# alibaba/EasyParallelLibrary

Measured on AMD Instinct MI355X. Metric: samples_per_sec, higher is better.
Workload: dtype bf16; 1 GPU; model=bert-large, global_batch=128, seq_len=512, parallelism=dp1

## Files before the change

### csrc/bindings.hip

```cpp

#include <hip/hip_runtime.h>
#include <torch/extension.h>
#include <ATen/hip/impl/HIPStreamMasqueradingAsCUDA.h>

#include <cstdint>

namespace epl {
void register_comm(py::module& m);
}

extern "C" {
void epl_fused_adamw(float*, unsigned short*, const void*, bool, float*,
                     float*, int64_t, float, float, float, float, float, int,
                     float, hipStream_t);
void epl_lamb_phase1(const float*, const void*, bool, float*, float*, float*,
                     const int*, float*, float*, int64_t, float, float, float,
                     float, int, float, hipStream_t);
void epl_lamb_phase2(float*, unsigned short*, const float*, const int*,
                     const float*, int64_t, float, hipStream_t);
void epl_layer_norm_fwd(void*, const void*, const void*, void*, const void*,
                        const void*, float*, float*, int64_t, int64_t, float,
                        bool, hipStream_t);
void epl_layer_norm_bwd(void*, float*, float*, const void*, const void*,
                        const void*, const float*, const float*, float*,
// ... 11 lines not shown
                       hipStream_t);
void epl_ce_rowstats(const void*, const int64_t*, float*, float*, float*,
                     int64_t, int64_t, int64_t, int64_t, bool, hipStream_t);
void epl_ce_backward(void*, const void*, const int64_t*, const float*,
                     const float*, const float*, int64_t, int64_t, int64_t,
                     int64_t, float, bool, hipStream_t);
void epl_scale(void*, int64_t, float, bool, hipStream_t);
void epl_f32_to_bf16(unsigned short*, const float*, int64_t, hipStream_t);
void epl_bf16_to_f32(float*, const unsigned short*, int64_t, hipStream_t);
void epl_sqnorm(const void*, int64_t, float*, bool, hipStream_t);
void epl_colsum(void*, const void*, float*, int64_t, int64_t, int64_t,
                bool, hipStream_t);
void run_mfma_probe(const unsigned short*, const unsigned short*, float*,
                    hipStream_t);
void run_tr_read_probe(short*, short*, int, hipStream_t);
void epl_moe_dispatch_fwd(void*, const void*, const int64_t*,
                          const int64_t*, const int64_t*, int64_t, int64_t,
                          int64_t, hipStream_t);
void epl_moe_dispatch_bwd(void*, const void*, const int64_t*,
                          const int64_t*, const int64_t*, int64_t, int64_t,
                          int64_t, int64_t, hipStream_t);
void epl_moe_combine_fwd(void*, const void*, const float*, const int64_t*,
                         const int64_t*, const int64_t*, int64_t, int64_t,
                         int64_t, int64_t, hipStream_t);
void epl_moe_combine_bwd(void*, float*, const void*, const void*,
                         const float*, const int64_t*, const int64_t*,
                         const int64_t*, int64_t, int64_t, int64_t,
                         hipStream_t);
int64_t epl_moe_router_waves(int64_t, int64_t);
void epl_moe_router_fwd(const void*, int64_t*, float*, float*, int64_t*,
// ... 405 lines not shown
}

void tr_read_probe(at::Tensor out_gather, at::Tensor out_tr,
                   int64_t head_dim) {
  TORCH_CHECK(head_dim == 64 || head_dim == 128, "head_dim must be 64|128");
  check(out_gather, at::kShort, "out_gather");
  check(out_tr, at::kShort, "out_tr");
  const int64_t n = 4 * (head_dim / 32) * 64 * 8;
  TORCH_CHECK(out_gather.numel() == n && out_tr.numel() == n,
              "probe outputs must hold ", n, " elements");
  run_tr_read_probe(reinterpret_cast<short*>(out_gather.data_ptr()),
                    reinterpret_cast<short*>(out_tr.data_ptr()),
                    (int)head_dim, cur_stream());
}

void mfma_probe(at::Tensor A, at::Tensor B, at::Tensor D) {
  check(A, at::kBFloat16, "A");
  check(B, at::kBFloat16, "B");
  check(D, at::kFloat, "D");
  run_mfma_probe(reinterpret_cast<const unsigned short*>(A.data_ptr()),
                 reinterpret_cast<const unsigned short*>(B.data_ptr()),
                 D.data_ptr<float>(), cur_stream());
}

static void check_idx(const at::Tensor& t, const char* name) {
  TORCH_CHECK(t.is_cuda() && t.is_contiguous() &&
              t.scalar_type() == at::kLong, name,
              " must be a contiguous int64 device tensor");
}

// ... 308 lines not shown
  m.def("layer_norm_bwd", &layer_norm_bwd);
  m.def("layer_norm_bwd_fused", &layer_norm_bwd_fused, py::arg("dx"),
        py::arg("dgamma"), py::arg("dbeta"), py::arg("dy"), py::arg("x"),
        py::arg("gamma"), py::arg("mean"), py::arg("rstd"),
        py::arg("dadd") = py::none(), py::arg("colsum_out") = py::none());
  m.def("bias_gelu_fwd", &bias_gelu_fwd);
  m.def("bias_gelu_bwd", &bias_gelu_bwd);
  m.def("ce_rowstats", &ce_rowstats);
  m.def("ce_backward", &ce_backward);
  m.def("scale_", &scale_);
  m.def("f32_to_bf16", &f32_to_bf16);
  m.def("bf16_to_f32", &bf16_to_f32);
  m.def("sqnorm", &sqnorm);
  m.def("mfma_probe", &mfma_probe);
  m.def("tr_read_probe", &tr_read_probe);
  m.def("moe_dispatch_fwd", &moe_dispatch_fwd);
  m.def("moe_dispatch_bwd", &moe_dispatch_bwd);
  m.def("moe_combine_fwd", &moe_combine_fwd);
  m.def("moe_combine_bwd", &moe_combine_bwd);
  m.def("moe_router_fwd", &moe_router_fwd);
  m.def("moe_router_bwd", &moe_router_bwd);
  m.def("moe_router_waves", [](int64_t n, int64_t e) {
    return epl_moe_router_waves(n, e);
  });
  m.def("attn_fwd", &attn_fwd, py::arg("q"), py::arg("k"), py::arg("v"),
        py::arg("out"), py::arg("lse"), py::arg("scale"), py::arg("causal"),
        py::arg("drop_mask"), py::arg("seed"), py::arg("drop_thresh"),
        py::arg("inv_keep"), py::arg("seqlens") = py::none());
  m.def("attn_bwd", &attn_bwd, py::arg("q"), py::arg("k"), py::arg("v"),
        py::arg("out"), py::arg("dout"), py::arg("lse"),
// ... 16 lines not shown
```

### csrc/kernels/attention.hip

```cpp

#include <hip/hip_runtime.h>
#include <cstdint>
#include <cstdlib>
#include <cstring>
#include <type_traits>

#include "attn_lds_image.h"

using bf16x8 = __attribute__((ext_vector_type(8))) short;
using bf16x4 = __attribute__((ext_vector_type(4))) short;
using f32x16 = __attribute__((ext_vector_type(16))) float;
using i32x2 = __attribute__((ext_vector_type(2))) int;
using u32x2 = __attribute__((ext_vector_type(2))) unsigned int;
using f32x2 = __attribute__((ext_vector_type(2))) float;
using f32x4 = __attribute__((ext_vector_type(4))) float;
using bf16v2 = __attribute__((ext_vector_type(2))) __bf16;

#define DEVI __device__ __forceinline__

namespace {

DEVI float bf2f(short u) {
  union { unsigned int i; float f; } v;
  v.i = ((unsigned int)(unsigned short)u) << 16;
// ... 72 lines not shown
};

DEVI void store_acc_bf16(short* p, const f32x16& acc, int hi) {
#pragma unroll
  for (int g = 0; g < 4; ++g) {
    u32x2 v = {cvt_pk_bf16(acc[4 * g], acc[4 * g + 1]),
               cvt_pk_bf16(acc[4 * g + 2], acc[4 * g + 3])};
    *reinterpret_cast<u32x2*>(p + 8 * g + 4 * hi) = v;
  }
}

DEVI int64_t sample_len(const int* seqlens, int64_t b, int64_t seq) {
  if (seqlens == nullptr) return seq;
  const int64_t n = __builtin_amdgcn_readfirstlane(seqlens[b]);
  return n < 0 ? 0 : (n > seq ? seq : n);
}

template <int D>
DEVI void zero_row(short* p, int hi) {
  const u32x2 z = {0u, 0u};
#pragma unroll
  for (int j = 0; j < D / 32; ++j)
#pragma unroll
    for (int g = 0; g < 4; ++g)
      *reinterpret_cast<u32x2*>(p + j * 32 + 8 * g + 4 * hi) = z;
}

DEVI void philox_round(unsigned int& c0, unsigned int& c1,
                       unsigned int& c2, unsigned int& c3,
                       unsigned int k0, unsigned int k1) {
// ... 119 lines not shown
    const short* __restrict__ q, const short* __restrict__ k,
    const short* __restrict__ v, short* __restrict__ out,
    float* __restrict__ lse, int64_t seq, float scale, int causal,
    int64_t heads, int64_t in_sb, int64_t in_sh, int64_t in_ss,
    int64_t o_sb, int64_t o_sh, int64_t o_ss,
    unsigned int* __restrict__ mask, int64_t mask_w,
    unsigned long long seed, int drop_thresh, float inv_keep,
    const int* __restrict__ seqlens) {
  __shared__ __attribute__((aligned(16))) short
      ldsV[2][64 * img_pitch<D>()];
  __shared__ __attribute__((aligned(16))) short ldsK[2][64][D + 8];
  const int lane = threadIdx.x & 63;
  const int wave = threadIdx.x >> 6;
  const int hi = lane >> 5;
  const int lq = lane & 31;
  const int64_t bh = causal ? (int64_t)blockIdx.x : (int64_t)blockIdx.y;
  const int64_t boff = (bh / heads) * in_sb + (bh % heads) * in_sh;
  const int64_t qb = causal ? (int64_t)gridDim.y - 1 - blockIdx.y
                            : (int64_t)blockIdx.x;
  const int64_t q0_blk = qb * 128;
  const int64_t q0 = q0_blk + wave * 32;
  const int64_t len = sample_len(seqlens, bh / heads, seq);
  const int64_t myq = q0 + lq;
  if (myq >= len && myq < seq) {
    zero_row<D>(out + (bh / heads) * o_sb + (bh % heads) * o_sh +
                    myq * o_ss, hi);
    if (hi == 0) lse[bh * seq + myq] = 0.f;
  }
  if (q0_blk >= len) return;
  const bool active = q0 < len;
  const short* qp = q + boff;
  const short* kp = k + boff;
  const short* vp = v + boff;

  const int64_t qrow = myq < len ? myq : len - 1;
// ... 97 lines not shown
#pragma unroll
  for (int j = 0; j < D / 32; ++j)
    store_acc_bf16(ldsO + lq * (D + 8) + j * 32, ot[j] * inv_l, hi);
  __syncthreads();
  constexpr int LPR = D / 8;
#pragma unroll
  for (int r0 = 0; r0 < 32; r0 += 64 / LPR) {
    const int r = r0 + lane / LPR;
    const int col = (lane % LPR) * 8;
    const bf16x8 piece =
        *reinterpret_cast<const bf16x8*>(ldsO + r * (D + 8) + col);
    if (q0 + r < len)
      *reinterpret_cast<bf16x8*>(ob + (q0 + r) * o_ss + col) = piece;
  }
  if (hi == 0 && myq < len) lse[bh * seq + myq] = m * scale + __logf(l);
}

__global__ void attn_bwd_prep_kernel(const short* __restrict__ dout,
                                     const short* __restrict__ out,
                                     float* __restrict__ delta,
                                     int64_t rows, int64_t seq,
                                     int64_t heads, int64_t do_sb,
                                     int64_t do_sh, int64_t do_ss,
                                     int64_t o_sb, int64_t o_sh,
                                     int64_t o_ss) {
  const int lane = threadIdx.x & 63;
  const int waves_per_block = blockDim.x >> 6;
  for (int64_t row = (int64_t)blockIdx.x * waves_per_block +
                     (threadIdx.x >> 6);
       row < rows; row += (int64_t)gridDim.x * waves_per_block) {
    const int64_t bh = row / seq;
    const int64_t sq = row % seq;
    const short* dp = dout + (bh / heads) * do_sb + (bh % heads) * do_sh +
                      sq * do_ss;
    const short* op = out + (bh / heads) * o_sb + (bh % heads) * o_sh +
                      sq * o_ss;
    float acc = bf2f(dp[lane]) * bf2f(op[lane]);
#pragma unroll
    for (int off = 32; off > 0; off >>= 1)
      acc += __shfl_down(acc, off, 64);
    if (lane == 0) delta[row] = acc;
  }
}

__global__ __launch_bounds__(256) void attn_bwd_dkdv_kernel(
    const short* __restrict__ q, const short* __restrict__ k,
    const short* __restrict__ v, const short* __restrict__ dout,
    const float* __restrict__ lse, const float* __restrict__ delta,
    short* __restrict__ dk, short* __restrict__ dv, int64_t seq,
    float scale, int causal, int64_t heads, int64_t in_sb, int64_t in_sh,
    int64_t in_ss, int64_t do_sb, int64_t do_sh, int64_t do_ss,
    int64_t g_sb, int64_t g_sh, int64_t g_ss) {
  __shared__ short ldsQ[32][72];
  __shared__ short ldsDO[32][72];
  const int lane = threadIdx.x & 63;
  const int wave = threadIdx.x >> 6;
  const int hi = lane >> 5;
  const int lkv = lane & 31;
  const int64_t bh = blockIdx.y;
  const int64_t kv0_blk = (int64_t)blockIdx.x * 128;
  const int64_t kv0 = kv0_blk + wave * 32;
  const bool active = kv0 < seq;
  const int64_t boff = (bh / heads) * in_sb + (bh % heads) * in_sh;
  const short* qp = q + boff;
  const short* kp = k + boff;
  const short* vp = v + boff;
  const short* dop = dout + (bh / heads) * do_sb + (bh % heads) * do_sh;
  const float* lsep = lse + bh * seq;
  const float* dltp = delta + bh * seq;

  const int64_t mykv = kv0 + lkv;
  const int64_t kvrow = mykv < seq ? mykv : seq - 1;

  bf16x8 kfrag[4], vfrag[4];
#pragma unroll
  for (int c = 0; c < 4; ++c) {
    kfrag[c] = *reinterpret_cast<const bf16x8*>(
        kp + kvrow * in_ss + hi * 8 + 16 * c);
    vfrag[c] = *reinterpret_cast<const bf16x8*>(
        vp + kvrow * in_ss + hi * 8 + 16 * c);
  }

  f32x16 dvt0 = {}, dvt1 = {};
  f32x16 dkt0 = {}, dkt1 = {};

  const int stage_row = threadIdx.x >> 3;
  const int stage_seg = (threadIdx.x & 7) * 8;
  const int64_t q_start = causal ? (kv0_blk / 32) * 32 : 0;
  for (int64_t q0 = q_start; q0 < seq; q0 += 32) {
    __syncthreads();
    {
      int64_t qr = q0 + stage_row;
      if (qr >= seq) qr = seq - 1;
      *reinterpret_cast<bf16x8*>(&ldsQ[stage_row][stage_seg]) =
          *reinterpret_cast<const bf16x8*>(qp + qr * in_ss + stage_seg);
      *reinterpret_cast<bf16x8*>(&ldsDO[stage_row][stage_seg]) =
          *reinterpret_cast<const bf16x8*>(dop + qr * do_ss + stage_seg);
    }
    __syncthreads();
    if (!active || (causal && q0 + 31 < kv0)) continue;
    f32x16 st = {};
    f32x16 dpt = {};
#pragma unroll
    for (int c = 0; c < 4; ++c) {
      bf16x8 qf = *reinterpret_cast<const bf16x8*>(
          &ldsQ[lkv][hi * 8 + 16 * c]);
      bf16x8 dof = *reinterpret_cast<const bf16x8*>(
          &ldsDO[lkv][hi * 8 + 16 * c]);
      st = __builtin_amdgcn_mfma_f32_32x32x16_bf16(qf, kfrag[c], st, 0, 0,
                                                   0);
      dpt = __builtin_amdgcn_mfma_f32_32x32x16_bf16(dof, vfrag[c], dpt, 0,
                                                    0, 0);
    }
    float p[16], ds[16];
#pragma unroll
    for (int r = 0; r < 16; ++r) {
      const int64_t qg = q0 + crow(r, hi);
      const int64_t qgc = qg < seq ? qg : seq - 1;
      float sv = st[r] * scale;
      bool masked = qg >= seq || (causal && mykv > qg) || mykv >= seq;
      float pv = masked ? 0.f : __expf(sv - lsep[qgc]);
      p[r] = pv;
      ds[r] = masked ? 0.f : pv * (dpt[r] - dltp[qgc]) * scale;
    }
    bf16x8 pb0 = assemble_pfrag(&p[0]);
    bf16x8 pb1 = assemble_pfrag(&p[8]);
    bf16x8 db0 = assemble_pfrag(&ds[0]);
    bf16x8 db1 = assemble_pfrag(&ds[8]);
#pragma unroll
    for (int qc = 0; qc < 2; ++qc) {
      bf16x8 dot0, dot1, qt0, qt1;
#pragma unroll
      for (int j = 0; j < 8; ++j) {
        const int qr = qc * 16 + hi * 8 + j;
        dot0[j] = ldsDO[qr][lkv];
        dot1[j] = ldsDO[qr][32 + lkv];
        qt0[j] = ldsQ[qr][lkv];
        qt1[j] = ldsQ[qr][32 + lkv];
      }
      bf16x8 pb = qc == 0 ? pb0 : pb1;
      bf16x8 db = qc == 0 ? db0 : db1;
      dvt0 = __builtin_amdgcn_mfma_f32_32x32x16_bf16(dot0, pb, dvt0, 0, 0,
                                                     0);
      dvt1 = __builtin_amdgcn_mfma_f32_32x32x16_bf16(dot1, pb, dvt1, 0, 0,
                                                     0);
      dkt0 = __builtin_amdgcn_mfma_f32_32x32x16_bf16(qt0, db, dkt0, 0, 0,
                                                     0);
      dkt1 = __builtin_amdgcn_mfma_f32_32x32x16_bf16(qt1, db, dkt1, 0, 0,
                                                     0);
    }
  }

  if (!active || mykv >= seq) return;
  const int64_t goff = (bh / heads) * g_sb + (bh % heads) * g_sh +
                       mykv * g_ss;
  short* dkp = dk + goff;
  short* dvp = dv + goff;
#pragma unroll
  for (int r = 0; r < 16; ++r) {
    dvp[crow(r, hi)] = (short)f2bf(dvt0[r]);
    dvp[32 + crow(r, hi)] = (short)f2bf(dvt1[r]);
    dkp[crow(r, hi)] = (short)f2bf(dkt0[r]);
    dkp[32 + crow(r, hi)] = (short)f2bf(dkt1[r]);
  }
}


template <bool MASKED, bool DROP, int D>
DEVI void dv_tile(const short (&ldsQ)[64][D + 8],
                  const short (&ldsDO)[64][D + 8],
                  int sub, int64_t q0, int64_t seq, int64_t mykv,
                  float scale, int causal, const float* lsep,
                  const bf16x8 (&kfrag)[D / 16], f32x16 (&dvt)[D / 32],
                  int lkv, int hi, const unsigned int* maskrow,
                  int64_t mask_w, float inv_keep) {
  f32x16 st = {};
#pragma unroll
  for (int c = 0; c < D / 16; ++c) {
    bf16x8 qf = *reinterpret_cast<const bf16x8*>(
// ... 209 lines not shown
    int64_t heads, int64_t in_sb, int64_t in_sh, int64_t in_ss,
    int64_t do_sb, int64_t do_sh, int64_t do_ss, int64_t g_sb,
    int64_t g_sh, int64_t g_ss,
    const unsigned int* __restrict__ mask, int64_t mask_w,
    float inv_keep, const int* __restrict__ seqlens) {
  constexpr int PITCH = TR ? img_pitch<D>() : D + 8;
  __shared__ __attribute__((aligned(16))) short
      ldsQ[DBUF ? 2 : 1][64][PITCH];
  __shared__ __attribute__((aligned(16))) short
      ldsDO[DBUF ? 2 : 1][64][PITCH];
  __shared__ __attribute__((aligned(16))) float ldsL[DBUF ? 2 : 1][64];
  const int lane = threadIdx.x & 63;
  const int wave = threadIdx.x >> 6;
  const int hi = lane >> 5;
  const int lkv = lane & 31;
  const int64_t bh = causal ? (int64_t)blockIdx.x : (int64_t)blockIdx.y;
  const int64_t kv0_blk =
      (causal ? (int64_t)blockIdx.y : (int64_t)blockIdx.x) * 128;
  const int64_t kv0 = kv0_blk + wave * 32;
  const int64_t len = sample_len(seqlens, bh / heads, seq);
  const int64_t mykv = kv0 + lkv;
  if (mykv >= len && mykv < seq)
    zero_row<D>(dv + (bh / heads) * g_sb + (bh % heads) * g_sh +
                    mykv * g_ss, hi);
  if (kv0_blk >= len) return;
  const bool active = kv0 < len;
  const int64_t boff = (bh / heads) * in_sb + (bh % heads) * in_sh;
  const short* qp = q + boff;
  const short* kp = k + boff;
  const short* dop = dout + (bh / heads) * do_sb + (bh % heads) * do_sh;
  const float* lsep = lse + bh * seq;

  const int64_t kvrow = mykv < len ? mykv : len - 1;
// ... 170 lines not shown
    int64_t heads, int64_t in_sb, int64_t in_sh, int64_t in_ss,
    int64_t do_sb, int64_t do_sh, int64_t do_ss, int64_t g_sb,
    int64_t g_sh, int64_t g_ss,
    const unsigned int* __restrict__ mask, int64_t mask_w,
    float inv_keep, const int* __restrict__ seqlens) {
  constexpr int PITCH = TR ? img_pitch<D>() : D + 8;
  __shared__ __attribute__((aligned(16))) short
      ldsQ[DBUF ? 2 : 1][64][PITCH];
  __shared__ __attribute__((aligned(16))) short
      ldsDO[DBUF ? 2 : 1][64][PITCH];
  __shared__ __attribute__((aligned(16))) float ldsL[DBUF ? 2 : 1][2][64];
  const int lane = threadIdx.x & 63;
  const int wave = threadIdx.x >> 6;
  const int hi = lane >> 5;
  const int lkv = lane & 31;
  const int64_t bh = causal ? (int64_t)blockIdx.x : (int64_t)blockIdx.y;
  const int64_t kv0_blk =
      (causal ? (int64_t)blockIdx.y : (int64_t)blockIdx.x) * 128;
  const int64_t kv0 = kv0_blk + wave * 32;
  const int64_t len = sample_len(seqlens, bh / heads, seq);
  const int64_t mykv = kv0 + lkv;
  if (mykv >= len && mykv < seq)
    zero_row<D>(dk + (bh / heads) * g_sb + (bh % heads) * g_sh +
                    mykv * g_ss, hi);
  if (kv0_blk >= len) return;
  const bool active = kv0 < len;
  const int64_t boff = (bh / heads) * in_sb + (bh % heads) * in_sh;
  const short* qp = q + boff;
  const short* kp = k + boff;
  const short* vp = v + boff;
  const short* dop = dout + (bh / heads) * do_sb + (bh % heads) * do_sh;
  const float* lsep = lse + bh * seq;
  const float* dltp = delta + bh * seq;
// ... 156 lines not shown
  if (!active || mykv >= len) return;
  short* dkp = dk + (bh / heads) * g_sb + (bh % heads) * g_sh +
               mykv * g_ss;
#pragma unroll
  for (int dj = 0; dj < D / 32; ++dj) {
    if constexpr (TR) {
      store_acc_bf16(dkp + dj * 32, dkt[dj], hi);
    } else {
#pragma unroll
      for (int r = 0; r < 16; ++r)
        dkp[dj * 32 + crow(r, hi)] = (short)f2bf(dkt[dj][r]);
    }
  }
}


template <bool MASKED, bool DROP, int D>
DEVI void dq_tile(const short (&ldsK)[64][D + 8],
                  const short (&ldsVr)[64][D + 8],
                  int sub, int64_t kv0, int64_t seq, int64_t myq,
                  float scale, int causal, float mylse, float mydelta,
                  const bf16x8 (&qfrag)[D / 16],
                  const bf16x8 (&dofrag)[D / 16],
                  f32x16 (&dqt)[D / 32], int lq, int hi,
                  const unsigned int* maskrow, int64_t mask_w,
                  float inv_keep) {
  f32x16 st = {};
  f32x16 dpt = {};
#pragma unroll
  for (int c = 0; c < D / 16; ++c) {
// ... 104 lines not shown
    float scale, int causal, int64_t heads, int64_t in_sb, int64_t in_sh,
    int64_t in_ss, int64_t do_sb, int64_t do_sh, int64_t do_ss,
    int64_t g_sb, int64_t g_sh, int64_t g_ss, int64_t o_sb, int64_t o_sh,
    int64_t o_ss, const unsigned int* __restrict__ mask, int64_t mask_w,
    float inv_keep, const float* __restrict__ dlse,
    const int* __restrict__ seqlens) {
  constexpr int PITCH = TR ? img_pitch<D>() : D + 8;
  __shared__ __attribute__((aligned(16))) short
      ldsK[DBUF ? 2 : 1][64][PITCH];
  __shared__ __attribute__((aligned(16))) short
      ldsVr[DBUF ? 2 : 1][64][PITCH];
  const int lane = threadIdx.x & 63;
  const int wave = threadIdx.x >> 6;
  const int hi = lane >> 5;
  const int lq = lane & 31;
  const int64_t bh = causal ? (int64_t)blockIdx.x : (int64_t)blockIdx.y;
  const int64_t qb = causal ? (int64_t)gridDim.y - 1 - blockIdx.y
                            : (int64_t)blockIdx.x;
  const int64_t q0_blk = qb * 128;
  const int64_t q0 = q0_blk + wave * 32;
  const int64_t len = sample_len(seqlens, bh / heads, seq);
  const int64_t myq = q0 + lq;
  if (myq >= len && myq < seq)
    zero_row<D>(dq + (bh / heads) * g_sb + (bh % heads) * g_sh +
                    myq * g_ss, hi);
  if (q0_blk >= len) return;
  const bool active = q0 < len;
  const int64_t boff = (bh / heads) * in_sb + (bh % heads) * in_sh;
  const short* qp = q + boff;
  const short* kp = k + boff;
  const short* vp = v + boff;
  const short* dop = dout + (bh / heads) * do_sb + (bh % heads) * do_sh;

  const int64_t qrow = myq < len ? myq : len - 1;
// ... 194 lines not shown
                       dim3(256), 0, stream, FWD_ARGS);
  }
#undef FWD_ARGS
}

void epl_attn_bwd(const void* q, const void* k, const void* v,
                  const void* out, const void* dout, const float* lse,
                  float* delta_ws, void* dq, void* dk, void* dv,
                  int64_t batch_heads, int64_t seq, float scale,
                  bool causal, int64_t heads, const int64_t* in_strides,
                  const int64_t* o_strides, const int64_t* do_strides,
                  const int64_t* g_strides, int split_dkdv,
                  const unsigned int* drop_mask, int64_t mask_w,
                  float inv_keep, int64_t head_dim, const float* dlse,
                  const int* seqlens, hipStream_t stream) {
  const int64_t rows = batch_heads * seq;
  const unsigned nqb = (unsigned)((seq + 127) / 128);
  dim3 grid = causal ? dim3((unsigned)batch_heads, nqb)
                     : dim3(nqb, (unsigned)batch_heads);
  if (split_dkdv || drop_mask != nullptr || head_dim == 128 || causal ||
      dlse != nullptr || seqlens != nullptr) {
#define DV_ARGS                                                          \
  reinterpret_cast<const short*>(q), reinterpret_cast<const short*>(k),  \
      reinterpret_cast<const short*>(dout), lse,                         \
      reinterpret_cast<short*>(dv), seq, scale, causal ? 1 : 0, heads,   \
      in_strides[0], in_strides[1], in_strides[2], do_strides[0],        \
      do_strides[1], do_strides[2], g_strides[0], g_strides[1],          \
      g_strides[2], drop_mask, mask_w, inv_keep, seqlens
#define DQ_ARGS                                                          \
  reinterpret_cast<const short*>(q), reinterpret_cast<const short*>(k),  \
      reinterpret_cast<const short*>(v),                                 \
      reinterpret_cast<const short*>(dout), lse, delta_ws,               \
      reinterpret_cast<short*>(dq), reinterpret_cast<const short*>(out), \
      seq, scale, causal ? 1 : 0, heads, in_strides[0], in_strides[1],   \
      in_strides[2], do_strides[0], do_strides[1], do_strides[2],        \
      g_strides[0], g_strides[1], g_strides[2], o_strides[0],            \
      o_strides[1], o_strides[2], drop_mask, mask_w, inv_keep, dlse,     \
// ... 10 lines not shown
      const char* e = getenv("EPL_ATTN_BWD_DBUF");
      return e == nullptr ? -1 : atoi(e);
    }();
    const int mode = dbuf_mode < 0 ? (causal ? 0 : 2) : dbuf_mode;
    const bool dbuf = mode >= 1;
    const bool dbuf_k = mode >= 2;
    const bool dbuf_q = mode >= 3;
    static const bool legacy_tiles = [] {
      const char* e = getenv("EPL_ATTN_BWD_TILES");
      return e != nullptr && strcmp(e, "legacy") == 0;
    }();
    auto launch3 = [&](auto drop_c, auto d_c, auto tr_c) {
      constexpr bool DROP = decltype(drop_c)::value;
      constexpr int D = decltype(d_c)::value;
      constexpr bool TR = decltype(tr_c)::value;
      if (D == 64 && dbuf)
        hipLaunchKernelGGL(
            HIP_KERNEL_NAME(attn_bwd_dv_kernel<DROP, D == 64, D, TR>), grid,
            dim3(256), 0, stream, DV_ARGS);
      else
        hipLaunchKernelGGL(
            HIP_KERNEL_NAME(attn_bwd_dv_kernel<DROP, false, D, TR>), grid,
            dim3(256), 0, stream, DV_ARGS);
      if (D == 64 && dbuf_q)
        hipLaunchKernelGGL(
            HIP_KERNEL_NAME(attn_bwd_dq_kernel<DROP, D == 64, D, TR>), grid,
            dim3(256), 0, stream, DQ_ARGS);
      else
        hipLaunchKernelGGL(
            HIP_KERNEL_NAME(attn_bwd_dq_kernel<DROP, false, D, TR>), grid,
            dim3(256), 0, stream, DQ_ARGS);
      if (D == 64 && dbuf_k)
        hipLaunchKernelGGL(
            HIP_KERNEL_NAME(attn_bwd_dk_kernel<DROP, D == 64, D, TR>), grid,
            dim3(256), 0, stream, DK_ARGS);
      else
        hipLaunchKernelGGL(
            HIP_KERNEL_NAME(attn_bwd_dk_kernel<DROP, false, D, TR>), grid,
            dim3(256), 0, stream, DK_ARGS);
    };
    auto launch2 = [&](auto drop_c, auto d_c) {
      if (legacy_tiles)
        launch3(drop_c, d_c, std::false_type{});
      else
        launch3(drop_c, d_c, std::true_type{});
    };
    using d64 = std::integral_constant<int, 64>;
    using d128 = std::integral_constant<int, 128>;
    if (head_dim == 128) {
      if (drop_mask != nullptr)
        launch2(std::true_type{}, d128{});
      else
        launch2(std::false_type{}, d128{});
    } else if (drop_mask != nullptr) {
      launch2(std::true_type{}, d64{});
    } else {
      launch2(std::false_type{}, d64{});
    }
#undef DV_ARGS
#undef DQ_ARGS
#undef DK_ARGS
    return;
  }
  {
    const int64_t blocks = (rows + 3) / 4;
    hipLaunchKernelGGL(attn_bwd_prep_kernel,
                       dim3((unsigned)(blocks < 4096 ? blocks : 4096)),
                       dim3(256), 0, stream,
                       reinterpret_cast<const short*>(dout),
                       reinterpret_cast<const short*>(out), delta_ws, rows,
                       seq, heads, do_strides[0], do_strides[1],
                       do_strides[2], o_strides[0], o_strides[1],
                       o_strides[2]);
  }
  hipLaunchKernelGGL(attn_bwd_dkdv_kernel, grid, dim3(256), 0, stream,
                     reinterpret_cast<const short*>(q),
                     reinterpret_cast<const short*>(k),
                     reinterpret_cast<const short*>(v),
                     reinterpret_cast<const short*>(dout), lse, delta_ws,
                     reinterpret_cast<short*>(dk),
                     reinterpret_cast<short*>(dv), seq, scale,
                     causal ? 1 : 0, heads, in_strides[0], in_strides[1],
                     in_strides[2], do_strides[0], do_strides[1],
                     do_strides[2], g_strides[0], g_strides[1],
                     g_strides[2]);
  hipLaunchKernelGGL(
      HIP_KERNEL_NAME(attn_bwd_dq_kernel<false, false, 64, true>),
                     grid, dim3(256), 0, stream,
                     reinterpret_cast<const short*>(q),
                     reinterpret_cast<const short*>(k),
                     reinterpret_cast<const short*>(v),
                     reinterpret_cast<const short*>(dout), lse, delta_ws,
                     reinterpret_cast<short*>(dq),
                     reinterpret_cast<const short*>(out), seq, scale,
                     causal ? 1 : 0, heads, in_strides[0], in_strides[1],
                     in_strides[2], do_strides[0], do_strides[1],
                     do_strides[2], g_strides[0], g_strides[1],
                     g_strides[2], o_strides[0], o_strides[1],
                     o_strides[2], drop_mask, mask_w, inv_keep, dlse,
                     (const int*)nullptr);
}

}
```

### csrc/kernels/mfma_probe.hip

```cpp

#include <hip/hip_runtime.h>

#include "attn_lds_image.h"

using bf16x8 = __attribute__((ext_vector_type(8))) short;
using f32x16 = __attribute__((ext_vector_type(16))) float;

__global__ void mfma_probe_kernel(const unsigned short* __restrict__ A,
                                  const unsigned short* __restrict__ B,
                                  float* __restrict__ D) {
  const int lane = threadIdx.x & 63;
  const int half = lane >> 5;
  const int lm = lane & 31;
  bf16x8 a, b;
  for (int j = 0; j < 8; ++j) {
    a[j] = (short)A[lm * 16 + (half * 8 + j)];
    b[j] = (short)B[(half * 8 + j) * 32 + lm];
  }
  f32x16 c = {};
  c = __builtin_amdgcn_mfma_f32_32x32x16_bf16(a, b, c, 0, 0, 0);
  for (int reg = 0; reg < 16; ++reg) {
    const int row = (reg & 3) + 8 * (reg >> 2) + 4 * half;
    const int col = lm;
    D[row * 32 + col] = c[reg];
// ... 28 lines not shown
        const bf16x8 t = attn_img::tr_frag<D>(img, sub + qc * 16, dj, lane);
        *reinterpret_cast<bf16x8*>(out_gather + (frag * 64 + lane) * 8) = g;
        *reinterpret_cast<bf16x8*>(out_tr + (frag * 64 + lane) * 8) = t;
      }
}

extern "C" void run_tr_read_probe(short* out_gather, short* out_tr,
                                  int head_dim, hipStream_t stream) {
  if (head_dim == 128)
    hipLaunchKernelGGL(tr_read_probe_kernel<128>, dim3(1), dim3(64), 0,
                       stream, out_gather, out_tr);
  else
    hipLaunchKernelGGL(tr_read_probe_kernel<64>, dim3(1), dim3(64), 0,
                       stream, out_gather, out_tr);
}
```

### easyparallellibrary_amd/ops/attention.py

```python

import torch
import torch.nn.functional as F

from easyparallellibrary_amd.ops.dispatch import native_ext, use_native
from easyparallellibrary_amd.utils.logging import get_logger

logger = get_logger()
_warned = set()


def _warn_fallback(reason):
    if reason not in _warned:
        _warned.add(reason)
        logger.warning(
            "native attention unavailable (%s): falling back to torch "
            "SDPA for these shapes", reason)


def _kernel_ok(t):
    return (t.dim() == 4 and t.shape[-1] in (64, 128)
            and t.stride(-1) == 1
            and t.stride(1) % 8 == 0 and t.stride(2) % 8 == 0)


# ... 14 lines not shown
    if seqlens is None:
        return None
    if seqlens.dtype != torch.int32 or seqlens.dim() != 1 \
            or seqlens.shape[0] != q.shape[0]:
        raise ValueError("seqlens must be int32 [B={}], got {} {}".format(
            q.shape[0], seqlens.dtype, tuple(seqlens.shape)))
    if seqlens.device != q.device:
        raise ValueError("seqlens must be on the device of q")
    return seqlens.contiguous()


def _mask_tensor(b, h, seq, device):
    mask_w = (seq + 31) // 32
    return torch.empty(b * h * seq * mask_w, dtype=torch.int32,
                       device=device)


def _saved_optionals(ctx, rest):
    rest = list(rest)
    mask = rest.pop(0) if ctx.has_mask else None
    seqlens = rest.pop(0) if ctx.has_seqlens else None
    return mask, seqlens


class _FlashAttention(torch.autograd.Function):

    @staticmethod
    def forward(ctx, q, k, v, causal, scale, dropout_p=0.0, seqlens=None):
        if not (_kernel_ok(q) and _kernel_ok(k) and _kernel_ok(v)
                and q.stride() == k.stride() == v.stride()):
# ... 6 lines not shown
        thresh, inv_keep, seed = _drop_params(dropout_p)
        mask = _mask_tensor(b, h, seq, q.device) if thresh else None
        native_ext().attn_fwd(q, k, v, out, lse, scale, causal, mask,
                              seed, thresh, inv_keep, seqlens)
        ctx.has_mask = mask is not None
        ctx.has_seqlens = seqlens is not None
        ctx.save_for_backward(q, k, v, out, lse, *[
            t for t in (mask, seqlens) if t is not None])
        ctx.causal = causal
        ctx.scale = scale
        ctx.inv_keep = inv_keep
        return out

    @staticmethod
    def backward(ctx, dout):
        import os
        saved = ctx.saved_tensors
        q, k, v, out, lse = saved[:5]
        mask, seqlens = _saved_optionals(ctx, saved[5:])
        orig_q = q
        contig = os.environ.get("EPL_ATTN_BWD_CONTIG", "0") == "1"
        if contig and q.stride(2) != 64:
            q, k, v = q.contiguous(), k.contiguous(), v.contiguous()
        if not _kernel_ok(dout) or (contig and dout.stride(2) != 64):
            dout = dout.contiguous()
        def grad_like(t):
            g = torch.empty_strided(t.shape, t.stride(), dtype=t.dtype,
                                    device=t.device)
            return g
        dq = grad_like(orig_q)
        dk = grad_like(orig_q)
        dv = grad_like(orig_q)
        delta = torch.empty_like(lse)
        split = os.environ.get("EPL_ATTN_BWD_SPLIT", "1") == "1"
        native_ext().attn_bwd(q, k, v, out, dout, lse, delta, dq, dk, dv,
                              ctx.scale, ctx.causal, split, mask,
                              ctx.inv_keep, None, seqlens)
        return dq, dk, dv, None, None, None, None


class _QKVFlashAttention(torch.autograd.Function):

    @staticmethod
    def forward(ctx, qkv, causal, scale, dropout_p=0.0, seqlens=None):
        b, s, three, h, d = qkv.shape
        q = qkv[:, :, 0].transpose(1, 2)
        k = qkv[:, :, 1].transpose(1, 2)
        v = qkv[:, :, 2].transpose(1, 2)
        out = torch.empty(b, s, h, d, dtype=qkv.dtype,
                          device=qkv.device).permute(0, 2, 1, 3)
        lse = torch.empty(b * h * s, dtype=torch.float32, device=qkv.device)
# ... 14 lines not shown
    def backward(ctx, dout):
        saved = ctx.saved_tensors
        qkv, out, lse = saved[:3]
        mask, seqlens = _saved_optionals(ctx, saved[3:])
        q = qkv[:, :, 0].transpose(1, 2)
        k = qkv[:, :, 1].transpose(1, 2)
        v = qkv[:, :, 2].transpose(1, 2)
        if not _kernel_ok(dout):
            dout = dout.contiguous()
        dqkv = torch.empty_like(qkv)
        dq = dqkv[:, :, 0].transpose(1, 2)
        dk = dqkv[:, :, 1].transpose(1, 2)
        dv = dqkv[:, :, 2].transpose(1, 2)
        delta = torch.empty_like(lse)
        native_ext().attn_bwd(q, k, v, out, dout, lse, delta, dq, dk, dv,
                              ctx.scale, ctx.causal, True, mask,
                              ctx.inv_keep, None, seqlens)
        return dqkv, None, None, None, None


class _FlashAttentionLse(torch.autograd.Function):

    @staticmethod
    def forward(ctx, q, k, v, causal, scale):
        if not (_kernel_ok(q) and _kernel_ok(k) and _kernel_ok(v)
                and q.stride() == k.stride() == v.stride()):
            q, k, v = q.contiguous(), k.contiguous(), v.contiguous()
        b, h, seq, d = q.shape
        out = torch.empty(b, seq, h, d, dtype=q.dtype,
                          device=q.device).permute(0, 2, 1, 3)
        lse = torch.empty(b * h * seq, dtype=torch.float32,
# ... 88 lines not shown
```

Before: 733.8 samples/s.

## Add fused pipelined dK/dV attention backward kernel and swizzled block order

Replaces the old simple dK/dV kernel with a new kernel that computes dK and dV in one pass. The new kernel double-buffers Q/dO tiles in an LDS image layout, prefetches the next tile from registers, reads transposed fragments from LDS and handles variable sequence lengths. The split backward becomes the default-off path, so the fused dK/dV kernel replaces separate dK and dV launches when there is no dropout, head_dim is 64 and attention is non-causal. Separately, non-causal forward and backward kernels now remap block indices so that groups of 8 heads are interleaved, aiming at better cache locality. The risk is that BERT training with attention dropout would skip the fused path, and the remapping could change L2 behaviour in either direction.

New measurement: 752.7 samples/s (median of 6 runs). 1.03x the previous value.

```diff
diff --git a/csrc/bindings.hip b/csrc/bindings.hip
--- a/csrc/bindings.hip
+++ b/csrc/bindings.hip
@@ -4,6 +4,8 @@
 #include <ATen/hip/impl/HIPStreamMasqueradingAsCUDA.h>
 
 #include <cstdint>
+
+#include "kernels/attn_block_order.h"
 
 namespace epl {
 void register_comm(py::module& m);
@@ -49,6 +51,7 @@
 void run_mfma_probe(const unsigned short*, const unsigned short*, float*,
                     hipStream_t);
 void run_tr_read_probe(short*, short*, int, hipStream_t);
+void run_block_order_probe(int*, int, int, hipStream_t);
 void epl_moe_dispatch_fwd(void*, const void*, const int64_t*,
                           const int64_t*, const int64_t*, int64_t, int64_t,
                           int64_t, hipStream_t);
@@ -484,6 +487,30 @@
                     (int)head_dim, cur_stream());
 }
 
+void attn_block_order_probe(at::Tensor out, int64_t n, int64_t bh) {
+  check(out, at::kInt, "out");
+  TORCH_CHECK(n >= 1 && n <= 65535 && bh >= 1 && bh <= 65535,
+              "grid dimensions must lie in [1, 65535]");
+  TORCH_CHECK(out.numel() == 2 * n * bh, "out must hold ", 2 * n * bh,
+              " elements");
+  run_block_order_probe(out.data_ptr<int>(), (int)n, (int)bh, cur_stream());
+}
+
+at::Tensor attn_block_order_host(int64_t n, int64_t bh) {
+  TORCH_CHECK(n >= 1 && n <= 65535 && bh >= 1 && bh <= 65535,
+              "grid dimensions must lie in [1, 65535]");
+  at::Tensor out = at::empty({n * bh, 2}, at::kInt);
+  int* p = out.data_ptr<int>();
+  for (int64_t y = 0; y < bh; ++y)
+    for (int64_t x = 0; x < n; ++x) {
+      const attn_order::Block b = attn_order::block_of(
+          (unsigned)x, (unsigned)y, (unsigned)n, (unsigned)bh);
+      p[2 * (x + n * y)] = (int)b.bh;
+      p[2 * (x + n * y) + 1] = (int)b.blk;
+    }
+  return out;
+}
+
 void mfma_probe(at::Tensor A, at::Tensor B, at::Tensor D) {
   check(A, at::kBFloat16, "A");
   check(B, at::kBFloat16, "B");
@@ -822,6 +849,8 @@
   m.def("sqnorm", &sqnorm);
   m.def("mfma_probe", &mfma_probe);
   m.def("tr_read_probe", &tr_read_probe);
+  m.def("attn_block_order_probe", &attn_block_order_probe);
+  m.def("attn_block_order_host", &attn_block_order_host);
   m.def("moe_dispatch_fwd", &moe_dispatch_fwd);
   m.def("moe_dispatch_bwd", &moe_dispatch_bwd);
   m.def("moe_combine_fwd", &moe_combine_fwd);
diff --git a/csrc/kernels/attention.hip b/csrc/kernels/attention.hip
--- a/csrc/kernels/attention.hip
+++ b/csrc/kernels/attention.hip
@@ -5,6 +5,7 @@
 #include <cstring>
 #include <type_traits>
 
+#include "attn_block_order.h"
 #include "attn_lds_image.h"
 
 using bf16x8 = __attribute__((ext_vector_type(8))) short;
@@ -110,6 +111,19 @@
   if (seqlens == nullptr) return seq;
   const int64_t n = __builtin_amdgcn_readfirstlane(seqlens[b]);
   return n < 0 ? 0 : (n > seq ? seq : n);
+}
+
+struct BlockPos {
+  int64_t bh, blk;
+};
+DEVI BlockPos block_pos(int causal, bool descending) {
+  if (causal)
+    return {(int64_t)blockIdx.x,
+            descending ? (int64_t)gridDim.y - 1 - blockIdx.y
+                       : (int64_t)blockIdx.y};
+  const attn_order::Block b =
+      attn_order::block_of(blockIdx.x, blockIdx.y, gridDim.x, gridDim.y);
+  return {(int64_t)b.bh, (int64_t)b.blk};
 }
 
 template <int D>
@@ -259,11 +273,10 @@
   const int wave = threadIdx.x >> 6;
   const int hi = lane >> 5;
   const int lq = lane & 31;
-  const int64_t bh = causal ? (int64_t)blockIdx.x : (int64_t)blockIdx.y;
+  const BlockPos pos = block_pos(causal, true);
+  const int64_t bh = pos.bh;
   const int64_t boff = (bh / heads) * in_sb + (bh % heads) * in_sh;
-  const int64_t qb = causal ? (int64_t)gridDim.y - 1 - blockIdx.y
-                            : (int64_t)blockIdx.x;
-  const int64_t q0_blk = qb * 128;
+  const int64_t q0_blk = pos.blk * 128;
   const int64_t q0 = q0_blk + wave * 32;
   const int64_t len = sample_len(seqlens, bh / heads, seq);
   const int64_t myq = q0 + lq;
@@ -391,155 +404,6 @@
       *reinterpret_cast<bf16x8*>(ob + (q0 + r) * o_ss + col) = piece;
   }
   if (hi == 0 && myq < len) lse[bh * seq + myq] = m * scale + __logf(l);
-}
-
-__global__ void attn_bwd_prep_kernel(const short* __restrict__ dout,
-                                     const short* __restrict__ out,
-                                     float* __restrict__ delta,
-                                     int64_t rows, int64_t seq,
-                                     int64_t heads, int64_t do_sb,
-                                     int64_t do_sh, int64_t do_ss,
-                                     int64_t o_sb, int64_t o_sh,
-                                     int64_t o_ss) {
-  const int lane = threadIdx.x & 63;
-  const int waves_per_block = blockDim.x >> 6;
-  for (int64_t row = (int64_t)blockIdx.x * waves_per_block +
-                     (threadIdx.x >> 6);
-       row < rows; row += (int64_t)gridDim.x * waves_per_block) {
-    const int64_t bh = row / seq;
-    const int64_t sq = row % seq;
-    const short* dp = dout + (bh / heads) * do_sb + (bh % heads) * do_sh +
-                      sq * do_ss;
-    const short* op = out + (bh / heads) * o_sb + (bh % heads) * o_sh +
-                      sq * o_ss;
-    float acc = bf2f(dp[lane]) * bf2f(op[lane]);
-#pragma unroll
-    for (int off = 32; off > 0; off >>= 1)
-      acc += __shfl_down(acc, off, 64);
-    if (lane == 0) delta[row] = acc;
-  }
-}
-
-__global__ __launch_bounds__(256) void attn_bwd_dkdv_kernel(
-    const short* __restrict__ q, const short* __restrict__ k,
-    const short* __restrict__ v, const short* __restrict__ dout,
-    const float* __restrict__ lse, const float* __restrict__ delta,
-    short* __restrict__ dk, short* __restrict__ dv, int64_t seq,
-    float scale, int causal, int64_t heads, int64_t in_sb, int64_t in_sh,
-    int64_t in_ss, int64_t do_sb, int64_t do_sh, int64_t do_ss,
-    int64_t g_sb, int64_t g_sh, int64_t g_ss) {
-  __shared__ short ldsQ[32][72];
-  __shared__ short ldsDO[32][72];
-  const int lane = threadIdx.x & 63;
-  const int wave = threadIdx.x >> 6;
-  const int hi = lane >> 5;
-  const int lkv = lane & 31;
-  const int64_t bh = blockIdx.y;
-  const int64_t kv0_blk = (int64_t)blockIdx.x * 128;
-  const int64_t kv0 = kv0_blk + wave * 32;
-  const bool active = kv0 < seq;
-  const int64_t boff = (bh / heads) * in_sb + (bh % heads) * in_sh;
-  const short* qp = q + boff;
-  const short* kp = k + boff;
-  const short* vp = v + boff;
-  const short* dop = dout + (bh / heads) * do_sb + (bh % heads) * do_sh;
-  const float* lsep = lse + bh * seq;
-  const float* dltp = delta + bh * seq;
-
-  const int64_t mykv = kv0 + lkv;
-  const int64_t kvrow = mykv < seq ? mykv : seq - 1;
-
-  bf16x8 kfrag[4], vfrag[4];
-#pragma unroll
-  for (int c = 0; c < 4; ++c) {
-    kfrag[c] = *reinterpret_cast<const bf16x8*>(
-        kp + kvrow * in_ss + hi * 8 + 16 * c);
-    vfrag[c] = *reinterpret_cast<const bf16x8*>(
-        vp + kvrow * in_ss + hi * 8 + 16 * c);
-  }
-
-  f32x16 dvt0 = {}, dvt1 = {};
-  f32x16 dkt0 = {}, dkt1 = {};
-
-  const int stage_row = threadIdx.x >> 3;
-  const int stage_seg = (threadIdx.x & 7) * 8;
-  const int64_t q_start = causal ? (kv0_blk / 32) * 32 : 0;
-  for (int64_t q0 = q_start; q0 < seq; q0 += 32) {
-    __syncthreads();
-    {
-      int64_t qr = q0 + stage_row;
-      if (qr >= seq) qr = seq - 1;
-      *reinterpret_cast<bf16x8*>(&ldsQ[stage_row][stage_seg]) =
-          *reinterpret_cast<const bf16x8*>(qp + qr * in_ss + stage_seg);
-      *reinterpret_cast<bf16x8*>(&ldsDO[stage_row][stage_seg]) =
-          *reinterpret_cast<const bf16x8*>(dop + qr * do_ss + stage_seg);
-    }
-    __syncthreads();
-    if (!active || (causal && q0 + 31 < kv0)) continue;
-    f32x16 st = {};
-    f32x16 dpt = {};
-#pragma unroll
-    for (int c = 0; c < 4; ++c) {
-      bf16x8 qf = *reinterpret_cast<const bf16x8*>(
-          &ldsQ[lkv][hi * 8 + 16 * c]);
-      bf16x8 dof = *reinterpret_cast<const bf16x8*>(
-          &ldsDO[lkv][hi * 8 + 16 * c]);
-      st = __builtin_amdgcn_mfma_f32_32x32x16_bf16(qf, kfrag[c], st, 0, 0,
-                                                   0);
-      dpt = __builtin_amdgcn_mfma_f32_32x32x16_bf16(dof, vfrag[c], dpt, 0,
-                                                    0, 0);
-    }
-    float p[16], ds[16];
-#pragma unroll
-    for (int r = 0; r < 16; ++r) {
-      const int64_t qg = q0 + crow(r, hi);
-      const int64_t qgc = qg < seq ? qg : seq - 1;
-      float sv = st[r] * scale;
-      bool masked = qg >= seq || (causal && mykv > qg) || mykv >= seq;
-      float pv = masked ? 0.f : __expf(sv - lsep[qgc]);
-      p[r] = pv;
-      ds[r] = masked ? 0.f : pv * (dpt[r] - dltp[qgc]) * scale;
-    }
-    bf16x8 pb0 = assemble_pfrag(&p[0]);
-    bf16x8 pb1 = assemble_pfrag(&p[8]);
-    bf16x8 db0 = assemble_pfrag(&ds[0]);
-    bf16x8 db1 = assemble_pfrag(&ds[8]);
-#pragma unroll
-    for (int qc = 0; qc < 2; ++qc) {
-      bf16x8 dot0, dot1, qt0, qt1;
-#pragma unroll
-      for (int j = 0; j < 8; ++j) {
-        const int qr = qc * 16 + hi * 8 + j;
-        dot0[j] = ldsDO[qr][lkv];
-        dot1[j] = ldsDO[qr][32 + lkv];
-        qt0[j] = ldsQ[qr][lkv];
-        qt1[j] = ldsQ[qr][32 + lkv];
-      }
-      bf16x8 pb = qc == 0 ? pb0 : pb1;
-      bf16x8 db = qc == 0 ? db0 : db1;
-      dvt0 = __builtin_amdgcn_mfma_f32_32x32x16_bf16(dot0, pb, dvt0, 0, 0,
-                                                     0);
-      dvt1 = __builtin_amdgcn_mfma_f32_32x32x16_bf16(dot1, pb, dvt1, 0, 0,
-                                                     0);
-      dkt0 = __builtin_amdgcn_mfma_f32_32x32x16_bf16(qt0, db, dkt0, 0, 0,
-                                                     0);
-      dkt1 = __builtin_amdgcn_mfma_f32_32x32x16_bf16(qt1, db, dkt1, 0, 0,
-                                                     0);
-    }
-  }
-
-  if (!active || mykv >= seq) return;
-  const int64_t goff = (bh / heads) * g_sb + (bh % heads) * g_sh +
-                       mykv * g_ss;
-  short* dkp = dk + goff;
-  short* dvp = dv + goff;
-#pragma unroll
-  for (int r = 0; r < 16; ++r) {
-    dvp[crow(r, hi)] = (short)f2bf(dvt0[r]);
-    dvp[32 + crow(r, hi)] = (short)f2bf(dvt1[r]);
-    dkp[crow(r, hi)] = (short)f2bf(dkt0[r]);
-    dkp[32 + crow(r, hi)] = (short)f2bf(dkt1[r]);
-  }
 }
 
 
@@ -779,9 +643,9 @@
   const int wave = threadIdx.x >> 6;
   const int hi = lane >> 5;
   const int lkv = lane & 31;
-  const int64_t bh = causal ? (int64_t)blockIdx.x : (int64_t)blockIdx.y;
-  const int64_t kv0_blk =
-      (causal ? (int64_t)blockIdx.y : (int64_t)blockIdx.x) * 128;
+  const BlockPos pos = block_pos(causal, false);
+  const int64_t bh = pos.bh;
+  const int64_t kv0_blk = pos.blk * 128;
   const int64_t kv0 = kv0_blk + wave * 32;
   const int64_t len = sample_len(seqlens, bh / heads, seq);
   const int64_t mykv = kv0 + lkv;
@@ -982,9 +846,9 @@
   const int wave = threadIdx.x >> 6;
   const int hi = lane >> 5;
   const int lkv = lane & 31;
-  const int64_t bh = causal ? (int64_t)blockIdx.x : (int64_t)blockIdx.y;
-  const int64_t kv0_blk =
-      (causal ? (int64_t)blockIdx.y : (int64_t)blockIdx.x) * 128;
+  const BlockPos pos = block_pos(causal, false);
+  const int64_t bh = pos.bh;
+  const int64_t kv0_blk = pos.blk * 128;
   const int64_t kv0 = kv0_blk + wave * 32;
   const int64_t len = sample_len(seqlens, bh / heads, seq);
   const int64_t mykv = kv0 + lkv;
@@ -1171,6 +1035,185 @@
   }
 }
 
+template <bool MASKED>
+DEVI void dkdv_tile_tr(const short* imgQ, const short* imgDO,
+                       const float* lseL, const float* dltL, int sub,
+                       int64_t q0, int64_t seq, int64_t mykv, float scale,
+                       const bf16x8 (&kfrag)[4], const bf16x8 (&vfrag)[4],
+                       f32x16 (&dvt)[2], f32x16 (&dkt)[2], int lkv, int hi) {
+  constexpr int D = 64;
+  f32x16 st = load_rowconst(lseL, hi);
+  f32x16 dpt = load_rowconst(dltL, hi);
+#pragma unroll
+  for (int c = 0; c < D / 16; ++c) {
+    const int o = img_off<D>(sub + lkv, 2 * c + hi);
+    bf16x8 qf = *reinterpret_cast<const bf16x8*>(imgQ + o);
+    bf16x8 dof = *reinterpret_cast<const bf16x8*>(imgDO + o);
+    st = __builtin_amdgcn_mfma_f32_32x32x16_bf16(qf, kfrag[c], st, 0, 0, 0);
+    dpt = __builtin_amdgcn_mfma_f32_32x32x16_bf16(dof, vfrag[c], dpt, 0, 0,
+                                                  0);
+  }
+  const float c2 = scale * 1.44269504088896341f;
+  const RowMask rm(q0, seq, mykv, 0);
+  float p[16], ds[16];
+#pragma unroll
+  for (int r = 0; r < 16; ++r) {
+    const float e = __builtin_amdgcn_exp2f(st[r] * c2);
+    if (MASKED) {
+      const bool m = rm.masked(crow(r, hi));
+      p[r] = m ? 0.f : e;
+      ds[r] = m ? 0.f : e * dpt[r] * scale;
+    } else {
+      p[r] = e;
+      ds[r] = e * dpt[r] * scale;
+    }
+  }
+  const int lane = hi * 32 + lkv;
+  bf16x8 pb0 = assemble_pfrag<true>(&p[0]);
+  bf16x8 pb1 = assemble_pfrag<true>(&p[8]);
+#pragma unroll
+  for (int qc = 0; qc < 2; ++qc) {
+    bf16x8 pb = qc == 0 ? pb0 : pb1;
+#pragma unroll
+    for (int dj = 0; dj < D / 32; ++dj) {
+      bf16x8 dot = tr_frag<D>(imgDO, sub + qc * 16, dj, lane);
+      dvt[dj] =
+          __builtin_amdgcn_mfma_f32_32x32x16_bf16(dot, pb, dvt[dj], 0, 0, 0);
+    }
+  }
+  bf16x8 db0 = assemble_pfrag<true>(&ds[0]);
+  bf16x8 db1 = assemble_pfrag<true>(&ds[8]);
+#pragma unroll
+  for (int qc = 0; qc < 2; ++qc) {
+    bf16x8 db = qc == 0 ? db0 : db1;
+#pragma unroll
+    for (int dj = 0; dj < D / 32; ++dj) {
+      bf16x8 qt = tr_frag<D>(imgQ, sub + qc * 16, dj, lane);
+      dkt[dj] =
+          __builtin_amdgcn_mfma_f32_32x32x16_bf16(qt, db, dkt[dj], 0, 0, 0);
+    }
+  }
+}
+
+__global__ __launch_bounds__(256, 2) void attn_bwd_dkdv_kernel(
+    const short* __restrict__ q, const short* __restrict__ k,
+    const short* __restrict__ v, const short* __restrict__ dout,
+    const float* __restrict__ lse, const float* __restrict__ delta,
+    short* __restrict__ dk, short* __restrict__ dv, int64_t seq,
+    float scale, int64_t heads, int64_t in_sb, int64_t in_sh,
+    int64_t in_ss, int64_t do_sb, int64_t do_sh, int64_t do_ss,
+    int64_t g_sb, int64_t g_sh, int64_t g_ss,
+    const int* __restrict__ seqlens) {
+  constexpr int D = 64;
+  __shared__ __attribute__((aligned(16))) short ldsQ[2][64][img_pitch<D>()];
+  __shared__ __attribute__((aligned(16))) short ldsDO[2][64][img_pitch<D>()];
+  __shared__ __attribute__((aligned(16))) float ldsL[2][2][64];
+  const int lane = threadIdx.x & 63;
+  const int wave = threadIdx.x >> 6;
+  const int hi = lane >> 5;
+  const int lkv = lane & 31;
+  const BlockPos pos = block_pos(0, false);
+  const int64_t bh = pos.bh;
+  const int64_t kv0_blk = pos.blk * 128;
+  const int64_t kv0 = kv0_blk + wave * 32;
+  const int64_t len = sample_len(seqlens, bh / heads, seq);
+  const int64_t mykv = kv0 + lkv;
+  const int64_t goff = (bh / heads) * g_sb + (bh % heads) * g_sh +
+                       mykv * g_ss;
+  if (mykv >= len && mykv < seq) {
+    zero_row<D>(dk + goff, hi);
+    zero_row<D>(dv + goff, hi);
+  }
+  if (kv0_blk >= len) return;
+  const bool active = kv0 < len;
+  const int64_t boff = (bh / heads) * in_sb + (bh % heads) * in_sh;
+  const short* qp = q + boff;
+  const short* kp = k + boff;
+  const short* vp = v + boff;
+  const short* dop = dout + (bh / heads) * do_sb + (bh % heads) * do_sh;
+  const float* lsep = lse + bh * seq;
+  const float* dltp = delta + bh * seq;
+
+  const int64_t kvrow = mykv < len ? mykv : len - 1;
+  bf16x8 kfrag[D / 16], vfrag[D / 16];
+#pragma unroll
+  for (int c = 0; c < D / 16; ++c) {
+    kfrag[c] = *reinterpret_cast<const bf16x8*>(
+        kp + kvrow * in_ss + hi * 8 + 16 * c);
+    vfrag[c] = *reinterpret_cast<const bf16x8*>(
+        vp + kvrow * in_ss + hi * 8 + 16 * c);
+  }
+
+  f32x16 dvt[D / 32] = {};
+  f32x16 dkt[D / 32] = {};
+  const int stage_row = threadIdx.x >> 3;
+  const int stage_seg = (threadIdx.x & 7) * 8;
+
+  bf16x8 rq[2], rdo[2];
+  float rl = 0.f;
+  const float neg_inv_scale = -1.f / scale;
+  auto prefetch = [&](int64_t q0) {
+    if (wave < 2) {
+      const int64_t qr = q0 + lane;
+      rl = (wave == 0 ? lsep : dltp)[qr < len ? qr : len - 1] *
+           (wave == 0 ? neg_inv_scale : -1.f);
+    }
+#pragma unroll
+    for (int half = 0; half < 2; ++half) {
+      int64_t qr = q0 + stage_row + half * 32;
+      if (qr >= len) qr = len - 1;
+      rq[half] = *reinterpret_cast<const bf16x8*>(qp + qr * in_ss +
+                                                  stage_seg);
+      rdo[half] = *reinterpret_cast<const bf16x8*>(dop + qr * do_ss +
+                                                   stage_seg);
+    }
+  };
+  auto commit = [&](int buf) {
+    if (wave < 2) ldsL[buf][wave][lane] = rl;
+#pragma unroll
+    for (int half = 0; half < 2; ++half) {
+      const int o = img_off<D>(stage_row + half * 32, stage_seg >> 3);
+      *reinterpret_cast<bf16x8*>(&ldsQ[buf][0][0] + o) = rq[half];
+      *reinterpret_cast<bf16x8*>(&ldsDO[buf][0][0] + o) = rdo[half];
+    }
+  };
+
+  const int64_t bulk_end = len & ~(int64_t)63;
+  int buf = 0;
+  prefetch(0);
+  for (int64_t q0 = 0; q0 < len; q0 += 64) {
+    commit(buf);
+    __syncthreads();
+    if (q0 + 64 < len) prefetch(q0 + 64);
+    const int rb = buf;
+    buf ^= 1;
+    const short* imgQ = &ldsQ[rb][0][0];
+    const short* imgDO = &ldsDO[rb][0][0];
+    if (q0 + 63 < bulk_end) {
+#pragma unroll
+      for (int sub = 0; sub < 64; sub += 32)
+        dkdv_tile_tr<false>(imgQ, imgDO, &ldsL[rb][0][sub],
+                            &ldsL[rb][1][sub], sub, q0 + sub, len, mykv,
+                            scale, kfrag, vfrag, dvt, dkt, lkv, hi);
+    } else if (active) {
+#pragma unroll
+      for (int sub = 0; sub < 64; sub += 32) {
+        const int64_t q0s = q0 + sub;
+        if (q0s >= len) break;
+        dkdv_tile_tr<true>(imgQ, imgDO, &ldsL[rb][0][sub],
+                           &ldsL[rb][1][sub], sub, q0s, len, mykv, scale,
+                           kfrag, vfrag, dvt, dkt, lkv, hi);
+      }
+    }
+  }
+  if (!active || mykv >= len) return;
+#pragma unroll
+  for (int dj = 0; dj < D / 32; ++dj) {
+    store_acc_bf16(dv + goff + dj * 32, dvt[dj], hi);
+    store_acc_bf16(dk + goff + dj * 32, dkt[dj], hi);
+  }
+}
+
 
 template <bool MASKED, bool DROP, int D>
 DEVI void dq_tile(const short (&ldsK)[64][D + 8],
@@ -1305,10 +1348,9 @@
   const int wave = threadIdx.x >> 6;
   const int hi = lane >> 5;
   const int lq = lane & 31;
-  const int64_t bh = causal ? (int64_t)blockIdx.x : (int64_t)blockIdx.y;
-  const int64_t qb = causal ? (int64_t)gridDim.y - 1 - blockIdx.y
-                            : (int64_t)blockIdx.x;
-  const int64_t q0_blk = qb * 128;
+  const BlockPos pos = block_pos(causal, true);
+  const int64_t bh = pos.bh;
+  const int64_t q0_blk = pos.blk * 128;
   const int64_t q0 = q0_blk + wave * 32;
   const int64_t len = sample_len(seqlens, bh / heads, seq);
   const int64_t myq = q0 + lq;
@@ -1533,13 +1575,13 @@
                   const unsigned int* drop_mask, int64_t mask_w,
                   float inv_keep, int64_t head_dim, const float* dlse,
                   const int* seqlens, hipStream_t stream) {
-  const int64_t rows = batch_heads * seq;
   const unsigned nqb = (unsigned)((seq + 127) / 128);
   dim3 grid = causal ? dim3((unsigned)batch_heads, nqb)
                      : dim3(nqb, (unsigned)batch_heads);
-  if (split_dkdv || drop_mask != nullptr || head_dim == 128 || causal ||
-      dlse != nullptr || seqlens != nullptr) {
-#define DV_ARGS                                                          \
+  const bool fused = !split_dkdv && drop_mask == nullptr &&
+                     head_dim == 64 && !causal;
+  {
+#define DV_ARGS                                                         \
   reinterpret_cast<const short*>(q), reinterpret_cast<const short*>(k),  \
       reinterpret_cast<const short*>(dout), lse,                         \
       reinterpret_cast<short*>(dv), seq, scale, causal ? 1 : 0, heads,   \
@@ -1580,7 +1622,8 @@
       constexpr bool DROP = decltype(drop_c)::value;
       constexpr int D = decltype(d_c)::value;
       constexpr bool TR = decltype(tr_c)::value;
-      if (D == 64 && dbuf)
+      if (fused) {
+      } else if (D == 64 && dbuf)
         hipLaunchKernelGGL(
             HIP_KERNEL_NAME(attn_bwd_dv_kernel<DROP, D == 64, D, TR>), grid,
             dim3(256), 0, stream, DV_ARGS);
@@ -1596,7 +1639,18 @@
         hipLaunchKernelGGL(
             HIP_KERNEL_NAME(attn_bwd_dq_kernel<DROP, false, D, TR>), grid,
             dim3(256), 0, stream, DQ_ARGS);
-      if (D == 64 && dbuf_k)
+      if (fused)
+        hipLaunchKernelGGL(
+            attn_bwd_dkdv_kernel, grid, dim3(256), 0, stream,
+            reinterpret_cast<const short*>(q),
+            reinterpret_cast<const short*>(k),
+            reinterpret_cast<const short*>(v),
+            reinterpret_cast<const short*>(dout), lse, delta_ws,
+            reinterpret_cast<short*>(dk), reinterpret_cast<short*>(dv), seq,
+            scale, heads, in_strides[0], in_strides[1], in_strides[2],
+            do_strides[0], do_strides[1], do_strides[2], g_strides[0],
+            g_strides[1], g_strides[2], seqlens);
+      else if (D == 64 && dbuf_k)
         hipLaunchKernelGGL(
             HIP_KERNEL_NAME(attn_bwd_dk_kernel<DROP, D == 64, D, TR>), grid,
             dim3(256), 0, stream, DK_ARGS);
@@ -1626,45 +1680,7 @@
 #undef DV_ARGS
 #undef DQ_ARGS
 #undef DK_ARGS
-    return;
-  }
-  {
-    const int64_t blocks = (rows + 3) / 4;
-    hipLaunchKernelGGL(attn_bwd_prep_kernel,
-                       dim3((unsigned)(blocks < 4096 ? blocks : 4096)),
-                       dim3(256), 0, stream,
-                       reinterpret_cast<const short*>(dout),
-                       reinterpret_cast<const short*>(out), delta_ws, rows,
-                       seq, heads, do_strides[0], do_strides[1],
-                       do_strides[2], o_strides[0], o_strides[1],
-                       o_strides[2]);
-  }
-  hipLaunchKernelGGL(attn_bwd_dkdv_kernel, grid, dim3(256), 0, stream,
-                     reinterpret_cast<const short*>(q),
-                     reinterpret_cast<const short*>(k),
-                     reinterpret_cast<const short*>(v),
-                     reinterpret_cast<const short*>(dout), lse, delta_ws,
-                     reinterpret_cast<short*>(dk),
-                     reinterpret_cast<short*>(dv), seq, scale,
-                     causal ? 1 : 0, heads, in_strides[0], in_strides[1],
-                     in_strides[2], do_strides[0], do_strides[1],
-                     do_strides[2], g_strides[0], g_strides[1],
-                     g_strides[2]);
-  hipLaunchKernelGGL(
-      HIP_KERNEL_NAME(attn_bwd_dq_kernel<false, false, 64, true>),
-                     grid, dim3(256), 0, stream,
-                     reinterpret_cast<const short*>(q),
-                     reinterpret_cast<const short*>(k),
-                     reinterpret_cast<const short*>(v),
-                     reinterpret_cast<const short*>(dout), lse, delta_ws,
-                     reinterpret_cast<short*>(dq),
-                     reinterpret_cast<const short*>(out), seq, scale,
-                     causal ? 1 : 0, heads, in_strides[0], in_strides[1],
-                     in_strides[2], do_strides[0], do_strides[1],
-                     do_strides[2], g_strides[0], g_strides[1],
-                     g_strides[2], o_strides[0], o_strides[1],
-                     o_strides[2], drop_mask, mask_w, inv_keep, dlse,
-                     (const int*)nullptr);
-}
-
-}
+  }
+}
+
+}
diff --git a/csrc/kernels/attn_block_order.h b/csrc/kernels/attn_block_order.h
--- /dev/null
+++ b/csrc/kernels/attn_block_order.h
@@ -0,0 +1,27 @@
+#pragma once
+
+#include <hip/hip_runtime.h>
+
+namespace attn_order {
+
+struct Block {
+  unsigned int bh, blk;
+};
+
+__host__ __device__ inline Block block_of(unsigned int x, unsigned int y,
+                                          unsigned int n, unsigned int BH) {
+  const unsigned int L = x + n * y;
+  const unsigned int BH8 = BH & ~7u;
+  Block b;
+  if (L < n * BH8) {
+    const unsigned int g = L & 7u, i = L >> 3;
+    b.blk = i % n;
+    b.bh = (i / n) * 8u + g;
+  } else {
+    b.bh = L / n;
+    b.blk = L % n;
+  }
+  return b;
+}
+
+}
diff --git a/csrc/kernels/mfma_probe.hip b/csrc/kernels/mfma_probe.hip
--- a/csrc/kernels/mfma_probe.hip
+++ b/csrc/kernels/mfma_probe.hip
@@ -1,6 +1,7 @@
 
 #include <hip/hip_runtime.h>
 
+#include "attn_block_order.h"
 #include "attn_lds_image.h"
 
 using bf16x8 = __attribute__((ext_vector_type(8))) short;
@@ -66,3 +67,18 @@
     hipLaunchKernelGGL(tr_read_probe_kernel<64>, dim3(1), dim3(64), 0,
                        stream, out_gather, out_tr);
 }
+
+__global__ void block_order_probe_kernel(int* __restrict__ out) {
+  if (threadIdx.x != 0) return;
+  const attn_order::Block b =
+      attn_order::block_of(blockIdx.x, blockIdx.y, gridDim.x, gridDim.y);
+  const unsigned int L = blockIdx.x + gridDim.x * blockIdx.y;
+  out[2 * (size_t)L] = (int)b.bh;
+  out[2 * (size_t)L + 1] = (int)b.blk;
+}
+
+extern "C" void run_block_order_probe(int* out, int n, int bh,
+                                      hipStream_t stream) {
+  hipLaunchKernelGGL(block_order_probe_kernel, dim3(n, bh), dim3(64), 0,
+                     stream, out);
+}
diff --git a/easyparallellibrary_amd/ops/attention.py b/easyparallellibrary_amd/ops/attention.py
--- a/easyparallellibrary_amd/ops/attention.py
+++ b/easyparallellibrary_amd/ops/attention.py
@@ -1,3 +1,5 @@
+
+import os
 
 import torch
 import torch.nn.functional as F
@@ -52,6 +54,10 @@
     mask_w = (seq + 31) // 32
     return torch.empty(b * h * seq * mask_w, dtype=torch.int32,
                        device=device)
+
+
+def _bwd_split():
+    return os.environ.get("EPL_ATTN_BWD_SPLIT", "0") == "1"
 
 
 def _saved_optionals(ctx, rest):
@@ -88,7 +94,6 @@
 
     @staticmethod
     def backward(ctx, dout):
-        import os
         saved = ctx.saved_tensors
         q, k, v, out, lse = saved[:5]
         mask, seqlens = _saved_optionals(ctx, saved[5:])
@@ -106,9 +111,8 @@
         dk = grad_like(orig_q)
         dv = grad_like(orig_q)
         delta = torch.empty_like(lse)
-        split = os.environ.get("EPL_ATTN_BWD_SPLIT", "1") == "1"
         native_ext().attn_bwd(q, k, v, out, dout, lse, delta, dq, dk, dv,
-                              ctx.scale, ctx.causal, split, mask,
+                              ctx.scale, ctx.causal, _bwd_split(), mask,
                               ctx.inv_keep, None, seqlens)
         return dq, dk, dv, None, None, None, None
 
@@ -153,7 +157,7 @@
         dv = dqkv[:, :, 2].transpose(1, 2)
         delta = torch.empty_like(lse)
         native_ext().attn_bwd(q, k, v, out, dout, lse, delta, dq, dk, dv,
-                              ctx.scale, ctx.causal, True, mask,
+                              ctx.scale, ctx.causal, _bwd_split(), mask,
                               ctx.inv_keep, None, seqlens)
         return dqkv, None, None, None, None
 
```
